# ilyakurdyukov/jpeg-quantsmooth

Measured on AMD Instinct MI355X. Metric: 8x8 blocks/s at q=3 niter=3, higher is better.
Workload: dtype f32

## Files before the change

### include/jpegqs_hip.h

```cpp
#ifndef JPEGQS_HIP_H
#define JPEGQS_HIP_H

#include <stddef.h>
#include <stdint.h>

#ifdef __cplusplus
extern "C" {
#endif

#define QS_HIP_MAXC 4

enum {
	QS_HIP_OK = 0,
	QS_HIP_ENODEV = -1,
	QS_HIP_EINVAL = -2,
	QS_HIP_ENOMEM = -3,
	QS_HIP_ENOTSUP = -4
};


typedef struct {
	int32_t ncomp;
	int32_t colorspace;
	int32_t image_width, image_height;
// ... 120 lines not shown
		int wblk, int hblk, int flags, int luma, int final_clamp, void *stream);
int qs_hip_smooth_plane_next(const void *d_consts, int16_t *d_coef, const uint8_t *d_plane, uint8_t *d_plane_next,
		int wblk, int hblk, int flags, int luma, int final_clamp, int rep_top, int rep_bot, void *stream);
int qs_hip_smooth_rows(const void *d_consts, int16_t *d_coef, const uint8_t *d_plane,
		int wblk, int hblk, int row0, int row1, int flags, int luma, int final_clamp, void *stream);

#define QS_HIP_MAX_PLANES 56
typedef struct {
	const void *d_consts;
	int16_t *d_coef;
	uint8_t *d_plane;
	int32_t *d_status;
	int32_t wblk, hblk, luma;
	int32_t band;
} qs_hip_plane_ref;
int qs_hip_idct_planes(const qs_hip_plane_ref *refs, int n, int first, void *stream);
int qs_hip_smooth_planes(const qs_hip_plane_ref *refs, int n, int flags, int final_clamp, void *stream);
int qs_hip_smooth_planes_next(const qs_hip_plane_ref *refs, uint8_t *const *d_plane_next, int n, int flags,
		int final_clamp, void *stream);

int qs_hip_joint_plane(const void *d_consts, int16_t *d_coef, const uint8_t *d_plane,
		const uint8_t *d_luma_lowres, int wblk, int hblk,
		int rebalance, int final_clamp, void *stream);
int qs_hip_lowq_plane(const void *d_consts, int16_t *d_coef, const uint8_t *d_plane,
		int wblk, int hblk, int rebalance, int final_clamp, void *stream);
int qs_hip_downsample_plane(const uint8_t *d_luma, int ywblk, int yhblk, uint8_t *d_lowres,
		int lwblk, int lhblk, int ws, int hs, void *stream);
size_t qs_hip_upsample_pitch(int image_width, int ws);
size_t qs_hip_upsample_bytes(int image_width, int image_height, int ws, int hs);
int qs_hip_upsample_plane(const uint8_t *d_chroma, const uint8_t *d_luma_lowres, int cwblk,
// ... 15 lines not shown
```

### jpeg-quantsmooth_amd/bands.py

```python
from __future__ import annotations

import os
from dataclasses import dataclass


_LIB = None


def _lib():
    global _LIB
    if _LIB is None:
        try:
            from .hipqs import HipQS
            _LIB = HipQS()
        except (OSError, RuntimeError, ImportError):
            _LIB = False
    return _LIB or None


def _band_rows_py(hblk: int, world: int, rank: int, align: int = 1):
    if hblk < 0 or world < 1 or not 0 <= rank < world or align < 1:
        raise ValueError("band_rows: bad argument")
    units = (hblk + align - 1) // align
    a, b = units * rank // world * align, units * (rank + 1) // world * align
# ... 162 lines not shown
        for w in dist.batch_isend_irecv(ops):
            w.wait()
    for dst_y, buf in recvs:
        view(dst_y).copy_(buf)


def run_bands_batched(engines, topo: BandTopology, niter: int, exchange_many) -> None:
    for it in range(niter):
        for e in engines:
            e.idct(it == 0, topo.rep_top, topo.rep_bot)
        exchange_many()
        for e in engines:
            e.smooth(it == niter - 1)


def run_bands_batched_sets(hip, engines, topo: BandTopology, niter: int, exchange_many, stream=None, mark=None, fused=True) -> None:
    band = (1 if topo.up is not None else 0) | (2 if topo.down is not None else 0)
    flags = engines[0].flags
    s = stream if stream is not None else engines[0]._s()
    if fused:
        for e in engines:
            e.ensure_plane2()
    for it in range(niter):
        if it == 0 or not fused:
            refs = hip.plane_refs([(e.cst.data_ptr(), e.coef.data_ptr(), e.plane.data_ptr(), e.status.data_ptr(),
                                    e.wblk, e.hblk, e.luma, band) for e in engines])
            hip.idct_planes(refs, it == 0, s)
        exchange_many()
        nxt = fused and it < niter - 1
        refs = hip.plane_refs([(e.cst.data_ptr(), e.coef.data_ptr(), e.plane.data_ptr(), e.status.data_ptr(),
                                e.wblk, e.hblk, e.luma, band, e.plane2.data_ptr() if nxt else None) for e in engines])
        if mark:
            mark(0)
        hip.smooth_planes(refs, flags, it == niter - 1, s)
        if mark:
            mark(1)
        if nxt:
            for e in engines:
                e.plane, e.plane2 = e.plane2, e.plane


def run_band_edge_first(hip, e, topo: BandTopology, niter: int, exchange, main, side, torch) -> None:
    if e.hblk < 3:
        return run_bands_batched_sets(hip, [e], topo, niter, exchange, stream=main.cuda_stream)
    e.ensure_plane2()
    band_top = 1 if topo.up is not None else 0
    band_bot = 2 if topo.down is not None else 0
    pitch, wb, hb = e.pitch, e.wblk, e.hblk
    row_bytes = wb * 128

    def views(cur, nxt):
        c0, p0 = e.coef.data_ptr(), cur.data_ptr()
        n0 = nxt.data_ptr() if nxt is not None else None
        at = lambda base, r: base + r * 8 * pitch if base is not None else None
        top = (e.cst.data_ptr(), c0, p0, e.status.data_ptr(), wb, 1, e.luma, band_top | 2, n0)
        bot = (e.cst.data_ptr(), c0 + (hb - 1) * row_bytes, at(p0, hb - 1), e.status.data_ptr(), wb, 1, e.luma, 1 | band_bot, at(n0, hb - 1))
        mid = (e.cst.data_ptr(), c0 + row_bytes, at(p0, 1), e.status.data_ptr(), wb, hb - 2, e.luma, 3, at(n0, 1))
        return hip.plane_refs([top, bot]), hip.plane_refs([mid])
    ev_main, ev_edge = torch.cuda.Event(), torch.cuda.Event()
    whole = hip.plane_refs([(e.cst.data_ptr(), e.coef.data_ptr(), e.plane.data_ptr(), e.status.data_ptr(), wb, hb, e.luma, band_top | band_bot)])
    hip.idct_planes(whole, True, main.cuda_stream)
    ev_main.record(main)
    side.wait_event(ev_main)
    with torch.cuda.stream(side):
        exchange()
    for it in range(niter):
        last = it == niter - 1
        edge, mid = views(e.plane, None if last else e.plane2)
        if it:
            side.wait_event(ev_main)
        hip.smooth_planes(edge, e.flags, last, side.cuda_stream)
        ev_edge_now = torch.cuda.Event(); ev_edge_now.record(side)
        if it:
            main.wait_event(ev_edge)
        hip.smooth_planes(mid, e.flags, last, main.cuda_stream)
        ev_main = torch.cuda.Event(); ev_main.record(main)
        ev_edge = ev_edge_now
        if not last:
            e.plane, e.plane2 = e.plane2, e.plane
            with torch.cuda.stream(side):
                exchange()
    main.wait_event(ev_edge)

# ... 379 lines not shown
```

### jpeg-quantsmooth_amd/csrc/qs_batch.cpp

```cpp
#include <functional>
#include <list>
#include <system_error>

#include "qs_jobint.h"

using namespace qsx;
using namespace qsj;

namespace {

static bool job_couplable(const qs_hip_job* job, int flags, int niter) {
  static const bool off = getenv("QS_HIP_NO_COUPLE") != nullptr;
  if (off || niter < 1 || (flags & QS_LOW_QUALITY) || !job_needs_lowres(job, flags)) return false;
  for (int ci = 0; ci < 3; ++ci) {
    if (!job->has_quant[ci]) return false;
    int acc = 0;
    for (int i = 0; i < 64; ++i) acc |= job->quant[ci][i];
    if (acc <= 1 || acc >= 0x800) return false;
  }
  return true;
}

struct ComputeSlots {
  std::mutex mu;
// ... 91 lines not shown
    for (int g = 0; g < G; ++g)
      for (int ci = 0; ci < 3; ++ci)
        host_pieces(jobs[which[g]], ci, 0, jobs[which[g]]->hblk[ci], cj[g].coef_off[ci], pieces);
    HIP_TRY(upload_pieces(coef.p, pieces, coef_bytes, s, stage));
  }
  HIP_TRY(hipMemsetAsync(status.p, 0, (size_t)G * 3 * sizeof(int32_t), s));
  ComputeSlot slot(current_device());

  auto coef_of = [&](int g, int ci) { return reinterpret_cast<int16_t*>(coef.as<char>() + cj[g].coef_off[ci]); };
  std::vector<unsigned char> cur((size_t)G * 3, 0);
  auto plane_at = [&](int g, int ci, int which_) {
    return px.as<uint8_t>() + cj[g].px_off[ci] + (which_ ? plane_stride(jobs[which[g]]->wblk[ci], jobs[which[g]]->hblk[ci]) : 0);
  };
  auto plane_of = [&](int g, int ci) { return plane_at(g, ci, cur[(size_t)g * 3 + ci]); };
  auto lowres_of = [&](int g) { return cj[g].sub ? px.as<uint8_t>() + cj[g].l_off : plane_of(g, 0); };
  auto make_set = [&](QsPlaneSet& set, int ci0, int ci1, const std::function<bool(int, int)>& next) {
    memset(&set, 0, sizeof set);
    int w = 0, n = 0;
    for (int g = 0; g < G; ++g)
      for (int ci = ci0; ci < ci1; ++ci, ++n) {
        const qs_hip_job* job = jobs[which[g]];
        set.wave0[n] = w;
        w += (job->wblk[ci] * job->hblk[ci] + 63) / 64;
        QsPlaneRef& R = set.ref[n];
        R.cst = cst.as<QsConsts>() + cj[g].cst[ci];
        R.coef = coef_of(g, ci);
        R.plane = plane_of(g, ci);
        R.plane_next = next(g, ci) ? plane_at(g, ci, !cur[(size_t)g * 3 + ci]) : nullptr;
        R.status = status.as<int32_t>() + g * 3 + ci;
        R.wblk = job->wblk[ci]; R.hblk = job->hblk[ci]; R.pitch = qs_plane_pitch(job->wblk[ci]);
        R.mode = QS_PLANE_REP_TOP | QS_PLANE_REP_BOT | (comp_rebalance(job, ci, flags) ? QS_PLANE_REBALANCE : 0);
      }
    set.n = n;
    for (int i = n; i < QS_MAX_PLANES + 2; ++i) set.wave0[i] = w;
  };
  auto flip = [&](int ci0, int ci1, const std::function<bool(int, int)>& next) {
    for (int g = 0; g < G; ++g) for (int ci = ci0; ci < ci1; ++ci) if (next(g, ci)) cur[(size_t)g * 3 + ci] ^= 1;
  };
  const std::function<bool(int, int)> none = [](int, int) { return false; }, all = [](int, int) { return true; };
  QsPlaneSet set;

  make_set(set, 0, 1, none);
  qs_launch_idct_set(set, 1, s);
  for (int it = 0; it < niter; ++it) {
    make_set(set, 0, 1, all);
    qs_launch_smooth_set(set, diag, it == niter - 1, s);
    flip(0, 1, all);
  }
  for (int g = 0; g < G; ++g) {
    const qs_hip_job* job = jobs[which[g]];
    if (cj[g].sub)
      qs_launch_downsample(plane_of(g, 0), job->wblk[0], job->hblk[0], lowres_of(g), job->wblk[1], job->hblk[1],
                           job->hsamp[0], job->vsamp[0], s);
  }

  QsPlaneAux lowres;
  memset(&lowres, 0, sizeof lowres);
  for (int g = 0; g < G; ++g) lowres.p[2 * g] = lowres.p[2 * g + 1] = lowres_of(g);
  bool any_up = false;
  for (int g = 0; g < G; ++g) any_up |= cj[g].upsample;
  const std::function<bool(int, int)> ups = [&](int g, int) { return cj[g].upsample; };
  make_set(set, 1, 3, none);
  qs_launch_idct_set(set, 1, s);
  for (int it = 0; it < niter; ++it) {
    const std::function<bool(int, int)>& next = it < niter - 1 ? all : ups;
    make_set(set, 1, 3, next);
    if (joint)
      qs_launch_joint_set(set, lowres, 0, 0, s);
    qs_launch_smooth_set(set, diag, it == niter - 1, s);
    flip(1, 3, next);
  }
  if (any_up) {
    for (int g = 0; g < G; ++g) {
      if (!cj[g].upsample) continue;
      const qs_hip_job* job = jobs[which[g]];
      const int ws = job->hsamp[0], hs = job->vsamp[0];
      const int w1 = (job->image_width + ws - 1) / ws, h1 = (job->image_height + hs - 1) / hs;
      const size_t pitch = qs_hip_upsample_pitch(job->image_width, ws);
      for (int k = 0; k < 2; ++k) {
        uint8_t* opx = upx.as<uint8_t>() + cj[g].upx_off[k];
        int16_t* oc = reinterpret_cast<int16_t*>(upc.as<char>() + cj[g].upc_off[k]);
// ... 198 lines not shown
```

### jpeg-quantsmooth_amd/csrc/qs_devfn.h

```cpp
#pragma once
#include <hip/hip_runtime.h>
#include <stdint.h>
#include "qs_device.h"

__device__ __forceinline__ int f2i_x86(float v) {
  return (v >= -2147483648.0f && v < 2147483648.0f) ? (int)v : (int)0x80000000;
}

__device__ __forceinline__ float round_half_away(float x) {
  float t = __builtin_truncf(x);
  float fr = __builtin_fabsf(x - t);
  return fr >= 0.5f ? t + __builtin_copysignf(1.0f, x) : t;
}

__device__ __forceinline__ void interval(int c, int div, int x1, int sh, int& orig, int& lo, int& hi) {
  int a = ((x1 * c) >> 16) + c;
  a = (int)(((uint32_t)a << sh) + 0x4000u) >> 15;
  a *= div;
  const int d0 = (div - 1) >> 1, d1 = div >> 1;
  orig = a;
  hi = a + (a < 0 ? d1 : d0);
  lo = a - (a > 0 ? d1 : d0);
}


__device__ __forceinline__ int qs_set_find(const QsPlaneSet& set, int w) {
  int lo = 0, hi = set.n - 1;
  while (lo < hi) {
    const int mid = (lo + hi + 1) >> 1;
    if (set.wave0[mid] <= w) lo = mid; else hi = mid - 1;
  }
  return lo;
}
```

### jpeg-quantsmooth_amd/csrc/qs_device.h

```cpp
#pragma once
#include <stdint.h>

#define QS_APRON_X 16
#define QS_LDS_PITCH 65
#define QS_TAB_MAX 272

enum {
  QS_DIAGONALS = 1, QS_JOINT_YUV = 2, QS_UPSAMPLE_UV = 4, QS_LOW_QUALITY = 8,
  QS_NO_REBALANCE = 16, QS_NO_REBALANCE_UV = 32, QS_TRANSCODE = 64
};

struct QsConsts {
  int32_t nat[64];
  int32_t q[64];
  int32_t qraw[64];
  int32_t x1[64];
  int32_t x2[64];
  float   range[64];
  int32_t qn[64], x1n[64], x2n[64];
  int32_t tab_size;
  int32_t pad[15];
  float   tab[64 * QS_TAB_MAX];
  int32_t rec[64][4];
};
// ... 14 lines not shown
}

#define QS_MAX_PLANES 56
struct QsPlaneRef {
  const QsConsts* cst;
  int16_t* coef;
  uint8_t* plane;
  int32_t* status;
  int32_t wblk, hblk, pitch;
  int32_t mode;
  uint8_t* plane_next;
};
enum {
  QS_PLANE_REBALANCE = 1,
  QS_PLANE_REP_TOP = 2,
  QS_PLANE_REP_BOT = 4
};
struct QsPlaneAux {
  const uint8_t* p[QS_MAX_PLANES];
};
struct QsPlaneSet {
  int32_t n, pad;
  int32_t wave0[QS_MAX_PLANES + 2];
  QsPlaneRef ref[QS_MAX_PLANES];
};
```

### jpeg-quantsmooth_amd/csrc/qs_device_job.cpp

```cpp
#include "qs_common.h"
#include "qs_device_job.h"

#include <algorithm>
#include <new>
#include <vector>

namespace {

size_t align_up(size_t n) { return (n + 255) & ~(size_t)255; }

struct DevComp {
  bool modified = false;
  bool passes = false;
  bool fuse = false;
  bool upsample = false;
  int iters = 0, extra = 0;
  size_t off_cst = 0, off_status = 0, off_plane = 0, off_plane2 = 0, off_snap = 0;
  bool snap = false;
};

struct DevPlan {
  int todo = 0;
  int niter = 0;
  int need_lowres = 0;
// ... 331 lines not shown
  return QS_HIP_OK;
}

int run_sets(qs_hip_job* const* jobs, int njobs, int flags, const BatchPlan& B, char* ws, hipStream_t s) {
  struct Id { int job, ci; };
  std::vector<unsigned char> cur((size_t)njobs * QS_HIP_MAXC, 0);
  auto plane_at = [&](const Id& d, int which) {
    const DevComp& C = B.P[d.job].c[d.ci];
    return reinterpret_cast<uint8_t*>(ws + B.region[d.job] + (which ? C.off_plane2 : C.off_plane));
  };
  auto plane_of = [&](const Id& d) { return plane_at(d, cur[(size_t)d.job * QS_HIP_MAXC + d.ci]); };
  auto lowres_of = [&](int i) {
    return B.P[i].llow_own ? reinterpret_cast<uint8_t*>(ws + B.region[i] + B.P[i].off_llow) : plane_of(Id{i, 0});
  };
  const int diag = (flags & QS_DIAGONALS) != 0;
  auto stage = [&](const std::vector<Id>& ids, bool idct, bool joint, int final_clamp, auto next) {
    for (size_t c0 = 0; c0 < ids.size(); c0 += QS_MAX_PLANES) {
      QsPlaneSet set;
      QsPlaneAux aux;
      memset(&set, 0, sizeof set);
      memset(&aux, 0, sizeof aux);
      const int n = (int)std::min<size_t>(QS_MAX_PLANES, ids.size() - c0);
      int w = 0;
      for (int k = 0; k < n; ++k) {
        const Id& d = ids[c0 + k];
        const qs_hip_job* job = jobs[d.job];
        const DevComp& C = B.P[d.job].c[d.ci];
        set.wave0[k] = w;
        w += (job->wblk[d.ci] * job->hblk[d.ci] + 63) / 64;
        QsPlaneRef& R = set.ref[k];
        R.cst = reinterpret_cast<const QsConsts*>(ws + B.region[d.job] + C.off_cst);
        R.coef = job->coef[d.ci];
        R.plane = plane_of(d);
        R.plane_next = !idct && next(d) ? plane_at(d, !cur[(size_t)d.job * QS_HIP_MAXC + d.ci]) : nullptr;
        R.status = reinterpret_cast<int32_t*>(ws + B.region[d.job] + C.off_status);
        R.wblk = job->wblk[d.ci]; R.hblk = job->hblk[d.ci]; R.pitch = qs_plane_pitch(job->wblk[d.ci]);
        const int rebalance = !(flags & QS_NO_REBALANCE) && (comp_luma(job, d.ci) || !(flags & QS_NO_REBALANCE_UV));
        R.mode = QS_PLANE_REP_TOP | QS_PLANE_REP_BOT | (rebalance ? QS_PLANE_REBALANCE : 0);
        aux.p[k] = lowres_of(d.job);
      }
      set.n = n;
      for (int k = n; k < QS_MAX_PLANES + 2; ++k) set.wave0[k] = w;
      if (idct) {
        qs_launch_idct_set(set, 1, s);
      } else {
        if (joint) qs_launch_joint_set(set, aux, 0, 0, s);
        qs_launch_smooth_set(set, diag, final_clamp, s);
      }
    }
    if (!idct)
      for (const Id& d : ids) if (next(d)) cur[(size_t)d.job * QS_HIP_MAXC + d.ci] ^= 1;
  };

  std::vector<Id> first, chroma;
  for (int i = 0; i < njobs; ++i) {
    if (B.route[i] == ROUTE_SET) for (int ci = 0; ci < jobs[i]->ncomp; ++ci) first.push_back({i, ci});
    if (B.route[i] == ROUTE_COUPLED) { first.push_back({i, 0}); chroma.push_back({i, 1}); chroma.push_back({i, 2}); }
  }
  int niter = 0;
  for (int i = 0; i < njobs; ++i) if (B.route[i] != ROUTE_SEQ) niter = B.P[i].niter;
  const auto none = [](const Id&) { return false; };

  stage(first, true, false, 0, none);
  for (int it = 0; it < niter; ++it) {
    const bool last = it == niter - 1;
    stage(first, false, false, last, [&](const Id& d) { return !last || B.route[d.job] == ROUTE_COUPLED; });
  }
  if (chroma.empty()) return QS_HIP_OK;
  for (int i = 0; i < njobs; ++i) {
    if (B.route[i] != ROUTE_COUPLED || !B.P[i].llow_own) continue;
    const qs_hip_job* job = jobs[i];
    if (int r = qs_hip_downsample_plane(plane_of(Id{i, 0}), job->wblk[0], job->hblk[0], lowres_of(i), job->wblk[1],
                                        job->hblk[1], job->hsamp[0], job->vsamp[0], s)) return r;
  }
  const bool joint = (flags & QS_JOINT_YUV) != 0;
  stage(chroma, true, false, 0, none);
  for (int it = 0; it < niter; ++it) {
    const bool last = it == niter - 1;
    stage(chroma, false, joint, last, [&](const Id& d) { return !last || B.P[d.job].c[d.ci].upsample; });
  }
  for (int i = 0; i < njobs; ++i) {
    if (B.route[i] != ROUTE_COUPLED || !B.P[i].up) continue;
    qs_hip_job* job = jobs[i];
    const int ws0 = job->hsamp[0], hs0 = job->vsamp[0];
    uint8_t* px = reinterpret_cast<uint8_t*>(ws + B.region[i] + B.P[i].off_px);
    for (int ci = 1; ci < 3; ++ci) {
      if (int r = qs_hip_upsample_plane(plane_of(Id{i, ci}), lowres_of(i), job->wblk[ci], plane_of(Id{i, 0}),
                                        job->wblk[0], job->hblk[0], px, job->image_width, job->image_height, ws0, hs0, s))
        return r;
      if (int r = qs_hip_fdct_plane(px, qs_hip_upsample_pitch(job->image_width, ws0), job->coef_up[ci - 1],
                                    job->wblk[0], job->hblk[0], s)) return r;
    }
  }
  return QS_HIP_OK;
// ... 143 lines not shown
```

### jpeg-quantsmooth_amd/csrc/qs_fused.cpp

```cpp
#include <list>

#include "qs_jobint.h"

using namespace qsx;
using namespace qsj;


namespace {
static size_t plane_stride(int wb, int hb) { return (qs_hip_plane_bytes(wb, hb) + 255) & ~(size_t)255; }
struct FPlane { int job, ci, wb, hb, cst; size_t coef_off, px_off, cbytes; int src_row0, keep0, keep1; };
struct FGroup {
  std::vector<FPlane> planes;
  std::vector<int> jobs;
  DevBuf coef, px, cst, status;
  PinnedBuf stage;
  std::vector<QsConsts> hc;
  PinnedBuf hstatus;
  Download down;
  hipStream_t s = nullptr;
  size_t blocks = 0, coef_bytes = 0;
  std::vector<hipEvent_t> it_ev;
  long long units = 0;
  PinnedBuf hstatus0;
  hipEvent_t ev_status0 = nullptr;
// ... 150 lines not shown
    set.n = np;
    int w = 0;
    for (int i = 0; i < np; ++i) {
      const FPlane& P = G.planes[i];
      set.wave0[i] = w;
      w += (P.wb * P.hb + 63) / 64;
      QsPlaneRef& R = set.ref[i];
      R.cst = G.cst.as<QsConsts>() + P.cst;
      R.coef = reinterpret_cast<int16_t*>(G.coef.as<char>() + P.coef_off);
      R.plane = G.px.as<uint8_t>() + P.px_off;
      R.status = G.status.as<int32_t>() + i;
      R.wblk = P.wb; R.hblk = P.hb; R.pitch = qs_plane_pitch(P.wb);
      R.mode = QS_PLANE_REP_TOP | QS_PLANE_REP_BOT | (comp_rebalance(jobs[P.job], P.ci, flags) ? QS_PLANE_REBALANCE : 0);
    }
    for (int i = np; i < QS_MAX_PLANES + 2; ++i) set.wave0[i] = w;
    qs_launch_idct_set(set, 1, G.s);
    if (plan) {
      if (!G.hstatus0.alloc((size_t)np * sizeof(int32_t))) return qs_fail(QS_HIP_ENOMEM, "out of pinned host memory");
      HIP_TRY(hipMemcpyAsync(G.hstatus0.p, G.status.p, (size_t)np * sizeof(int32_t), hipMemcpyDeviceToHost, G.s));
      HIP_TRY(hipEventCreateWithFlags(&G.ev_status0, hipEventDisableTiming));
      HIP_TRY(hipEventRecord(G.ev_status0, G.s));
    }
    for (int it = 0; it < niter; ++it) {
      for (int i = 0; i < np; ++i) {
        uint8_t* a = G.px.as<uint8_t>() + G.planes[i].px_off;
        uint8_t* b = a + plane_stride(G.planes[i].wb, G.planes[i].hb);
        set.ref[i].plane = (it & 1) ? b : a;
        set.ref[i].plane_next = it == niter - 1 ? nullptr : (it & 1) ? a : b;
      }
      qs_launch_smooth_set(set, diag, it == niter - 1, G.s);
      if (plan) {
        hipEvent_t e = nullptr;
        HIP_TRY(hipEventCreateWithFlags(&e, hipEventDisableTiming));
        G.it_ev.push_back(e);
        HIP_TRY(hipEventRecord(e, G.s));
      }
    }
    if (plan) for (const FPlane& P : G.planes) G.units += (long long)(P.keep1 - P.keep0) * jobs[P.job]->vsamp[P.ci];
    HIP_TRY(hipGetLastError());
    if (G.tev[1]) HIP_TRY(hipEventRecord(G.tev[1], G.s));
    if (!G.hstatus.alloc((size_t)np * sizeof(int32_t))) return qs_fail(QS_HIP_ENOMEM, "out of pinned host memory");
    HIP_TRY(hipMemcpyAsync(G.hstatus.p, G.status.p, (size_t)np * sizeof(int32_t), hipMemcpyDeviceToHost, G.s));
    HIP_TRY(G.down.issue(G.coef.p, coef_bytes, G.s, rows_active()));
    if (G.tev[2]) HIP_TRY(hipEventRecord(G.tev[2], G.s));
    if (!G.stage.p) for (int ji : G.jobs) if (split[ji]) defer[ji] = 1;
// ... 114 lines not shown
```

### jpeg-quantsmooth_amd/csrc/qs_kernels.hip

```cpp
#include <hip/hip_runtime.h>
#include <stdint.h>
#include <stdlib.h>
#include "qs_device.h"



__device__ __forceinline__ void wave_lds_sync() {
  __builtin_amdgcn_fence(__ATOMIC_RELEASE, "wavefront");
  __builtin_amdgcn_wave_barrier();
  __builtin_amdgcn_fence(__ATOMIC_ACQUIRE, "wavefront");
}

__device__ __forceinline__ uint32_t mulc(uint32_t a, int c) {
  return (uint32_t)__mul24((int)a, c);
}

__device__ __forceinline__ uint32_t lshl13_add(uint32_t x, uint32_t b) {
  uint32_t r;
  asm("v_lshl_add_u32 %0, %1, 13, %2" : "=v"(r) : "v"(x), "v"(b));
  return r;
}

__device__ __forceinline__ void idct8(uint32_t (&v)[8], uint32_t bias) {
  uint32_t z1, z2, z3, z4, z5, t0, t1, t2, t3, e0, e1, e2, e3;
// ... 85 lines not shown
                 int rep_top, int rep_bot, int blk) {
  const int by = blk / wblk, bx = blk - by * wblk;
  idct_pass1(ws);
  uint8_t* org = plane + (size_t)(by * 8 + 1) * pitch + QS_APRON_X + bx * 8;
#pragma unroll
  for (int y = 0; y < 8; ++y) {
    uint32_t row[8]; int o[8];
#pragma unroll
    for (int j = 0; j < 8; ++j) row[j] = ws[y * 8 + j];
    idct_pass2_row(row, o);
    store_pixel_row(org, pitch, y, o, bx, by, wblk, hblk, rep_top, rep_bot);
  }
}

__device__ __forceinline__ void
idct_block_to_plane(const QsConsts* __restrict__ cst, int16_t* __restrict__ coef,
                    uint8_t* __restrict__ plane, int wblk, int hblk, int pitch,
                    int first, int rep_top, int rep_bot, int* __restrict__ status, int blk) {
  uint4* cp = reinterpret_cast<uint4*>(coef) + (size_t)blk * 8;
  uint32_t ws[64];
#pragma unroll
  for (int j = 0; j < 8; ++j) {
    uint4 v = cp[j];
    uint32_t d[4] = {v.x, v.y, v.z, v.w};
#pragma unroll
    for (int c = 0; c < 4; ++c) {
      ws[j * 8 + c * 2] = (uint32_t)(int32_t)(int16_t)(d[c] & 0xffff);
      ws[j * 8 + c * 2 + 1] = (uint32_t)((int32_t)d[c] >> 16);
    }
  }
  if (first) {
    int bad = 0;
#pragma unroll
    for (int j = 0; j < 8; ++j) {
      uint32_t d[4];
#pragma unroll
      for (int c = 0; c < 4; ++c) {
        int lo = (int32_t)ws[j * 8 + c * 2] * cst->qraw[j * 8 + c * 2];
        int hi = (int32_t)ws[j * 8 + c * 2 + 1] * cst->qraw[j * 8 + c * 2 + 1];
        bad |= ((unsigned)(lo + 0x800) > 0xfffu) | ((unsigned)(hi + 0x800) > 0xfffu);
        lo = (int16_t)lo; hi = (int16_t)hi;
        ws[j * 8 + c * 2] = (uint32_t)lo; ws[j * 8 + c * 2 + 1] = (uint32_t)hi;
        d[c] = ((uint32_t)lo & 0xffffu) | ((uint32_t)hi << 16);
      }
      cp[j] = make_uint4(d[0], d[1], d[2], d[3]);
    }
    if (bad) atomicOr(status, 1);
  }
  idct_ws_to_plane(ws, plane, wblk, hblk, pitch, rep_top, rep_bot, blk);
}

__global__ void __launch_bounds__(256)
qs_idct_plane_kernel(const QsConsts* __restrict__ cst, int16_t* __restrict__ coef,
                     uint8_t* __restrict__ plane, int wblk, int hblk, int pitch,
                     int first, int rep_top, int rep_bot, int* __restrict__ status) {
  const int blk = blockIdx.x * 256 + threadIdx.x;
  if (blk >= wblk * hblk) return;
  idct_block_to_plane(cst, coef, plane, wblk, hblk, pitch, first, rep_top, rep_bot, status, blk);
}

#include "qs_devfn.h"

__global__ void __launch_bounds__(256)
qs_idct_set_kernel(const QsPlaneSet set, int first) {
  const int w = __builtin_amdgcn_readfirstlane((int)(blockIdx.x * 4 + (threadIdx.x >> 6)));
  if (w >= set.wave0[set.n]) return;
  const int i = qs_set_find(set, w);
  const QsPlaneRef& r = set.ref[i];
  const int blk = (w - set.wave0[i]) * 64 + (threadIdx.x & 63);
  if (blk >= r.wblk * r.hblk) return;
  idct_block_to_plane(r.cst, r.coef, r.plane, r.wblk, r.hblk, r.pitch, first,
                      r.mode & QS_PLANE_REP_TOP, r.mode & QS_PLANE_REP_BOT, r.status, blk);
}



typedef int16_t __attribute__((may_alias)) lds_i16;
__device__ __forceinline__ int lds_coef(const uint32_t* col, int i) {
  const lds_i16* p = reinterpret_cast<const lds_i16*>(col + (i >> 1) * QS_LDS_PITCH) + (i & 1);
  return *p;
}
__device__ __forceinline__ void lds_set_coef(uint32_t* col, int i, int v) {
  lds_i16* p = reinterpret_cast<lds_i16*>(col + (i >> 1) * QS_LDS_PITCH) + (i & 1);
  *p = (lds_i16)v;
}

static_assert(QS_LDS_PITCH * 4 == 260, "the literal offsets below assume a 260-byte row pitch");
// ... 143 lines not shown
#pragma unroll
    for (int c = 0; c < 4; ++c) {
      int lo = (int16_t)(d[c] & 0xffff), hi = (int32_t)d[c] >> 16;
      lo *= cst->qraw[j * 8 + c * 2]; hi *= cst->qraw[j * 8 + c * 2 + 1];
      d[c] = ((uint32_t)lo & 0xffffu) | ((uint32_t)hi << 16);
    }
    p[i] = make_uint4(d[0], d[1], d[2], d[3]);
  }
}

#include "qs_launch.h"

void qs_launch_idct_plane(const QsConsts* cst, int16_t* coef, uint8_t* plane, int wblk, int hblk,
                          int first, int rep_top, int rep_bot, int* status, hipStream_t s) {
  const int nblk = wblk * hblk;
  hipLaunchKernelGGL(qs_idct_plane_kernel, dim3((nblk + 255) / 256), dim3(256), 0, s,
                     cst, coef, plane, wblk, hblk, qs_plane_pitch(wblk), first, rep_top, rep_bot, status);
}

#define QS_DP_WAVES 4
static int qs_dp_waves(int groups) {
  static const int on = [] { const char* v = getenv("QS_HIP_DP"); return v ? atoi(v) : 1; }();
  static const int lim = [] { const char* v = getenv("QS_HIP_DP_GROUPS"); return v ? atoi(v) : 768; }();
  static const int lim2 = [] { const char* v = getenv("QS_HIP_DP_GROUPS2"); return v ? atoi(v) : 1536; }();
  if (!on) return 0;
  return groups <= lim ? QS_DP_WAVES : groups <= lim2 ? 2 : 0;
}

void qs_launch_smooth_plane(const QsConsts* cst, int16_t* coef, const uint8_t* plane, uint8_t* plane_next, int rep_top, int rep_bot,
                            int wblk, int hblk, int diag, int rebalance, int final_clamp, int blk_begin, int blk_end, hipStream_t s) {
  const int n = blk_end - blk_begin;
  if (n <= 0) return;
// ... 51 lines not shown
```

### jpeg-quantsmooth_amd/csrc/qs_planes.cpp

```cpp
#include "qs_common.h"


static int check_plane_args(const void* a, const void* b, int wblk, int hblk, const char* who) {
  if (!a || !b) return qs_fail(QS_HIP_EINVAL, "%s: null device pointer", who);
  if (wblk <= 0 || hblk <= 0 || (long long)wblk * hblk > (1ll << 28))
    return qs_fail(QS_HIP_EINVAL, "%s: bad plane size %dx%d blocks", who, wblk, hblk);
  return 0;
}


extern "C" int qs_hip_band_rows(int hblk, int nbands, int band, int align, int* row0, int* row1) {
  if (hblk < 0 || nbands < 1 || band < 0 || band >= nbands || align < 1 || !row0 || !row1)
    return qs_fail(QS_HIP_EINVAL, "qs_hip_band_rows: bad argument");
  const long long units = ((long long)hblk + align - 1) / align;
  const long long a = units * band / nbands * align, b = units * (band + 1) / nbands * align;
  *row0 = (int)(a < hblk ? a : hblk);
  *row1 = (int)(b < hblk ? b : hblk);
  return QS_HIP_OK;
}

extern "C" int qs_hip_colour_band_rows(int hblk_luma, int hblk_chroma, int v_samp, int nbands, int band,
                                       int* y0, int* y1, int* c0, int* c1) {
  if (v_samp < 1 || !y0 || !y1 || !c0 || !c1) return qs_fail(QS_HIP_EINVAL, "qs_hip_colour_band_rows: bad argument");
  if (int r = qs_hip_band_rows(hblk_chroma, nbands, band, 1, c0, c1)) return r;
// ... 69 lines not shown
  int w = 0;
  for (int i = 0; i < n; ++i) {
    const qs_hip_plane_ref& r = refs[i];
    if (int e = check_plane_args(r.d_coef, r.d_plane, r.wblk, r.hblk, who)) return e;
    if (!r.d_consts) return qs_fail(QS_HIP_EINVAL, "%s: null consts", who);
    set.wave0[i] = w;
    w += (r.wblk * r.hblk + 63) / 64;
    QsPlaneRef& R = set.ref[i];
    R.cst = static_cast<const QsConsts*>(r.d_consts);
    R.coef = r.d_coef; R.plane = r.d_plane; R.status = r.d_status;
    R.plane_next = next ? next[i] : nullptr;
    if (R.plane_next && R.plane_next == r.d_plane)
      return qs_fail(QS_HIP_EINVAL, "%s: d_plane_next must be a different buffer (other blocks still read d_plane)", who);
    R.wblk = r.wblk; R.hblk = r.hblk; R.pitch = qs_plane_pitch(r.wblk);
    R.mode = ((!(flags & QS_NO_REBALANCE) && (r.luma || !(flags & QS_NO_REBALANCE_UV))) ? QS_PLANE_REBALANCE : 0) |
             ((r.band & 1) ? 0 : QS_PLANE_REP_TOP) | ((r.band & 2) ? 0 : QS_PLANE_REP_BOT);
  }
  for (int i = n; i < QS_MAX_PLANES + 2; ++i) set.wave0[i] = w;
  return QS_HIP_OK;
}

extern "C" int qs_hip_idct_planes(const qs_hip_plane_ref* refs, int n, int first, void* stream) {
  QsPlaneSet set;
  if (int r = build_plane_set(refs, nullptr, n, 0, set, "qs_hip_idct_planes")) return r;
  if (first)
    for (int i = 0; i < n; ++i)
      if (!refs[i].d_status) return qs_fail(QS_HIP_EINVAL, "qs_hip_idct_planes: first pass needs d_status");
  qs_launch_idct_set(set, first, static_cast<hipStream_t>(stream));
  return launch_status("qs_hip_idct_planes");
}

// ... 97 lines not shown
```

### jpeg-quantsmooth_amd/csrc/qs_smooth_dp_kernel.inc

```
template <bool DIAG, int NW>
__global__ void __launch_bounds__(64 * NW, 3)
#ifdef QS_DP_SET
QS_DP_KERNEL_NAME(const QsPlaneSet set, int final_clamp) {
  const int gw = (int)blockIdx.x;
  if (gw >= set.wave0[set.n]) return;
  const int pi = qs_set_find(set, gw);
  const QsConsts* __restrict__ cst = set.ref[pi].cst;
  int16_t* __restrict__ coef = set.ref[pi].coef;
  const uint8_t* __restrict__ plane = set.ref[pi].plane;
  const int wblk = set.ref[pi].wblk, pitch = set.ref[pi].pitch;
  const int rebalance = set.ref[pi].mode & QS_PLANE_REBALANCE;
  const int nblk = wblk * set.ref[pi].hblk;
  const int base = (gw - set.wave0[pi]) * 64;
#else
QS_DP_KERNEL_NAME(const QsConsts* __restrict__ cst, int16_t* __restrict__ coef,
                  const uint8_t* __restrict__ plane, uint8_t* __restrict__ plane_next, int rep,
                  int wblk, int hblk, int pitch,
                  int rebalance, int final_clamp, int blk_begin, int blk_end) {
  const int nblk = blk_end;
  const int base = blk_begin + (int)blockIdx.x * 64;
#endif
  __shared__ uint32_t lds[32 * QS_LDS_PITCH];
  __shared__ long long reb_part[NW][64][2];
  __shared__ uint32_t chg_sh[3];
  __shared__ uint32_t ws_sh[64 * 64];
  const int lane = threadIdx.x & 63;
  const int wave = __builtin_amdgcn_readfirstlane((int)(threadIdx.x >> 6));
  uint32_t* col = lds + lane;
  if (blockDim.x != 64 * NW) __builtin_trap();
  if (base >= nblk) return;
  const int nvec = min(64, nblk - base) * 8;

  uint4* gsrc = reinterpret_cast<uint4*>(coef) + (size_t)base * 8;
  {
    const int m0 = (lane & 7) * 4;
#pragma unroll
    for (int j = 0; j < 8; ++j) {
      if (j % NW != wave) continue;
      const int idx = j * 64 + lane;
      uint4 v = make_uint4(0, 0, 0, 0);
      if (idx < nvec) v = gsrc[idx];
      uint32_t* dst = lds + m0 * QS_LDS_PITCH + (j * 8 + (lane >> 3));
      dst[0] = v.x; dst[QS_LDS_PITCH] = v.y; dst[2 * QS_LDS_PITCH] = v.z; dst[3 * QS_LDS_PITCH] = v.w;
    }
  }
  const int blk = min(base + lane, nblk - 1);
  const int by = blk / wblk, bx = blk - by * wblk;
  const uint8_t* org = plane + (size_t)(by * 8 + 1) * pitch + QS_APRON_X + bx * 8;
// ... 280 lines not shown
```

### jpeg-quantsmooth_amd/csrc/qs_smooth_kernel.inc

```
template <bool DIAG>
__global__ void __launch_bounds__(64 * QS_WAVES_PER_WG, QS_SMOOTH_MIN_WAVES)
#ifdef QS_SMOOTH_SET
QS_SMOOTH_KERNEL_NAME(const QsPlaneSet set, int final_clamp) {
  __shared__ uint32_t lds_all[QS_WAVES_PER_WG][32 * QS_LDS_PITCH];
#if QS_STASH
  __shared__ uint32_t stash_all[QS_WAVES_PER_WG][2 * 8 * 64];
#endif
  const int lane = threadIdx.x & 63, wave = threadIdx.x >> 6;
  uint32_t* lds = lds_all[wave];
  uint32_t* col = lds + lane;
  const int gw = __builtin_amdgcn_readfirstlane((int)(blockIdx.x * QS_WAVES_PER_WG + wave));
  if (gw >= set.wave0[set.n]) return;
  const int pi = qs_set_find(set, gw);
  const QsConsts* __restrict__ cst = set.ref[pi].cst;
  int16_t* __restrict__ coef = set.ref[pi].coef;
  const uint8_t* __restrict__ plane = set.ref[pi].plane;
  const int wblk = set.ref[pi].wblk, hblk = set.ref[pi].hblk, pitch = set.ref[pi].pitch;
  const int rebalance = set.ref[pi].mode & QS_PLANE_REBALANCE;
  const int nblk = wblk * hblk;
  const int base = (gw - set.wave0[pi]) * 64;
  (void)hblk;
#else
QS_SMOOTH_KERNEL_NAME(const QsConsts* __restrict__ cst, int16_t* __restrict__ coef,
                       const uint8_t* __restrict__ plane, uint8_t* __restrict__ plane_next, int rep,
// ... 6 lines not shown
  const int lane = threadIdx.x & 63, wave = threadIdx.x >> 6;
  uint32_t* lds = lds_all[wave];
  uint32_t* col = lds + lane;
  const int nblk = blk_end;
  const int base = blk_begin + (blockIdx.x * QS_WAVES_PER_WG + wave) * 64;
#endif
  if (base >= nblk) return;
  const int tail_prio = __builtin_amdgcn_readfirstlane(
      (gridDim.x > QS_RESIDENT_WG && blockIdx.x >= (gridDim.x / QS_RESIDENT_WG) * QS_RESIDENT_WG) ? 1 : 0);
  const int nvec = min(64, nblk - base) * 8;
#ifdef QS_STAGGER
  { unsigned hwid; asm volatile("s_getreg_b32 %0, hwreg(HW_REG_HW_ID)" : "=s"(hwid)); if (hwid & 1u) __builtin_amdgcn_s_sleep(QS_STAGGER); }
#endif

  uint4* gsrc = reinterpret_cast<uint4*>(coef) + (size_t)base * 8;
  {
    const int m0 = (lane & 7) * 4;
#pragma unroll
    for (int j = 0; j < 8; ++j) {
      const int idx = j * 64 + lane;
      uint4 v = make_uint4(0, 0, 0, 0);
      if (idx < nvec) v = gsrc[idx];
      uint32_t* dst = lds + m0 * QS_LDS_PITCH + (j * 8 + (lane >> 3));
      dst[0] = v.x; dst[QS_LDS_PITCH] = v.y; dst[2 * QS_LDS_PITCH] = v.z; dst[3 * QS_LDS_PITCH] = v.w;
    }
  }

  const int blk = min(base + lane, nblk - 1);
  const int by = blk / wblk, bx = blk - by * wblk;
  const uint8_t* org = plane + (size_t)(by * 8 + 1) * pitch + QS_APRON_X + bx * 8;
// ... 312 lines not shown
```

Baseline: 273.9 million.

## Defer first-pass dequantized coefficient writeback into first smooth pass; coalesce IDCT loads

The first IDCT pass no longer writes dequantized coefficients back to global memory when a smoothing pass follows. Instead, the first smooth kernel re-dequantizes the raw coefficients on load using a per-plane QS_PLANE_QUANT mode bit. The IDCT kernel is also restructured to load each wave's 64 blocks coalesced and transpose them through LDS, rather than having each thread read its own block. This removes one full coefficient write pass and improves load coalescing, at the cost of extra mode plumbing through every host path and a small dequant multiply in the first smooth pass.

```diff
diff --git a/include/jpegqs_hip.h b/include/jpegqs_hip.h
--- a/include/jpegqs_hip.h
+++ b/include/jpegqs_hip.h
@@ -158,6 +158,8 @@
 	int32_t wblk, hblk, luma;
 	int32_t band;
 } qs_hip_plane_ref;
+#define QS_HIP_PLANE_DEFER 4
+#define QS_HIP_FIRST_DEFER 2
 int qs_hip_idct_planes(const qs_hip_plane_ref *refs, int n, int first, void *stream);
 int qs_hip_smooth_planes(const qs_hip_plane_ref *refs, int n, int flags, int final_clamp, void *stream);
 int qs_hip_smooth_planes_next(const qs_hip_plane_ref *refs, uint8_t *const *d_plane_next, int n, int flags,
diff --git a/jpeg-quantsmooth_amd/bands.py b/jpeg-quantsmooth_amd/bands.py
--- a/jpeg-quantsmooth_amd/bands.py
+++ b/jpeg-quantsmooth_amd/bands.py
@@ -200,6 +200,10 @@
             e.smooth(it == niter - 1)
 
 
+def defer_bit() -> int:
+    return 0 if os.environ.get("QS_BANDS_DEFER", "1") == "0" else 4
+
+
 def run_bands_batched_sets(hip, engines, topo: BandTopology, niter: int, exchange_many, stream=None, mark=None, fused=True) -> None:
     band = (1 if topo.up is not None else 0) | (2 if topo.down is not None else 0)
     flags = engines[0].flags
@@ -208,14 +212,15 @@
         for e in engines:
             e.ensure_plane2()
     for it in range(niter):
+        q = defer_bit() if it == 0 else 0
         if it == 0 or not fused:
             refs = hip.plane_refs([(e.cst.data_ptr(), e.coef.data_ptr(), e.plane.data_ptr(), e.status.data_ptr(),
-                                    e.wblk, e.hblk, e.luma, band) for e in engines])
+                                    e.wblk, e.hblk, e.luma, band | q) for e in engines])
             hip.idct_planes(refs, it == 0, s)
         exchange_many()
         nxt = fused and it < niter - 1
         refs = hip.plane_refs([(e.cst.data_ptr(), e.coef.data_ptr(), e.plane.data_ptr(), e.status.data_ptr(),
-                                e.wblk, e.hblk, e.luma, band, e.plane2.data_ptr() if nxt else None) for e in engines])
+                                e.wblk, e.hblk, e.luma, band | q, e.plane2.data_ptr() if nxt else None) for e in engines])
         if mark:
             mark(0)
         hip.smooth_planes(refs, flags, it == niter - 1, s)
@@ -235,16 +240,17 @@
     pitch, wb, hb = e.pitch, e.wblk, e.hblk
     row_bytes = wb * 128
 
-    def views(cur, nxt):
+    def views(cur, nxt, q):
         c0, p0 = e.coef.data_ptr(), cur.data_ptr()
         n0 = nxt.data_ptr() if nxt is not None else None
         at = lambda base, r: base + r * 8 * pitch if base is not None else None
-        top = (e.cst.data_ptr(), c0, p0, e.status.data_ptr(), wb, 1, e.luma, band_top | 2, n0)
-        bot = (e.cst.data_ptr(), c0 + (hb - 1) * row_bytes, at(p0, hb - 1), e.status.data_ptr(), wb, 1, e.luma, 1 | band_bot, at(n0, hb - 1))
-        mid = (e.cst.data_ptr(), c0 + row_bytes, at(p0, 1), e.status.data_ptr(), wb, hb - 2, e.luma, 3, at(n0, 1))
+        top = (e.cst.data_ptr(), c0, p0, e.status.data_ptr(), wb, 1, e.luma, band_top | 2 | q, n0)
+        bot = (e.cst.data_ptr(), c0 + (hb - 1) * row_bytes, at(p0, hb - 1), e.status.data_ptr(), wb, 1, e.luma, 1 | band_bot | q, at(n0, hb - 1))
+        mid = (e.cst.data_ptr(), c0 + row_bytes, at(p0, 1), e.status.data_ptr(), wb, hb - 2, e.luma, 3 | q, at(n0, 1))
         return hip.plane_refs([top, bot]), hip.plane_refs([mid])
     ev_main, ev_edge = torch.cuda.Event(), torch.cuda.Event()
-    whole = hip.plane_refs([(e.cst.data_ptr(), e.coef.data_ptr(), e.plane.data_ptr(), e.status.data_ptr(), wb, hb, e.luma, band_top | band_bot)])
+    whole = hip.plane_refs([(e.cst.data_ptr(), e.coef.data_ptr(), e.plane.data_ptr(), e.status.data_ptr(), wb, hb, e.luma,
+                             band_top | band_bot | (defer_bit() if niter > 0 else 0))])
     hip.idct_planes(whole, True, main.cuda_stream)
     ev_main.record(main)
     side.wait_event(ev_main)
@@ -252,7 +258,7 @@
         exchange()
     for it in range(niter):
         last = it == niter - 1
-        edge, mid = views(e.plane, None if last else e.plane2)
+        edge, mid = views(e.plane, None if last else e.plane2, defer_bit() if it == 0 else 0)
         if it:
             side.wait_event(ev_main)
         hip.smooth_planes(edge, e.flags, last, side.cuda_stream)
diff --git a/jpeg-quantsmooth_amd/csrc/qs_batch.cpp b/jpeg-quantsmooth_amd/csrc/qs_batch.cpp
--- a/jpeg-quantsmooth_amd/csrc/qs_batch.cpp
+++ b/jpeg-quantsmooth_amd/csrc/qs_batch.cpp
@@ -129,7 +129,7 @@
   };
   auto plane_of = [&](int g, int ci) { return plane_at(g, ci, cur[(size_t)g * 3 + ci]); };
   auto lowres_of = [&](int g) { return cj[g].sub ? px.as<uint8_t>() + cj[g].l_off : plane_of(g, 0); };
-  auto make_set = [&](QsPlaneSet& set, int ci0, int ci1, const std::function<bool(int, int)>& next) {
+  auto make_set = [&](QsPlaneSet& set, int ci0, int ci1, const std::function<bool(int, int)>& next, bool quant = false) {
     memset(&set, 0, sizeof set);
     int w = 0, n = 0;
     for (int g = 0; g < G; ++g)
@@ -144,7 +144,8 @@
         R.plane_next = next(g, ci) ? plane_at(g, ci, !cur[(size_t)g * 3 + ci]) : nullptr;
         R.status = status.as<int32_t>() + g * 3 + ci;
         R.wblk = job->wblk[ci]; R.hblk = job->hblk[ci]; R.pitch = qs_plane_pitch(job->wblk[ci]);
-        R.mode = QS_PLANE_REP_TOP | QS_PLANE_REP_BOT | (comp_rebalance(job, ci, flags) ? QS_PLANE_REBALANCE : 0);
+        R.mode = QS_PLANE_REP_TOP | QS_PLANE_REP_BOT | (comp_rebalance(job, ci, flags) ? QS_PLANE_REBALANCE : 0) |
+                 (quant ? QS_PLANE_QUANT : 0);
       }
     set.n = n;
     for (int i = n; i < QS_MAX_PLANES + 2; ++i) set.wave0[i] = w;
@@ -155,10 +156,11 @@
   const std::function<bool(int, int)> none = [](int, int) { return false; }, all = [](int, int) { return true; };
   QsPlaneSet set;
 
-  make_set(set, 0, 1, none);
+  const bool defer_y = niter > 0;
+  make_set(set, 0, 1, none, defer_y);
   qs_launch_idct_set(set, 1, s);
   for (int it = 0; it < niter; ++it) {
-    make_set(set, 0, 1, all);
+    make_set(set, 0, 1, all, defer_y && it == 0);
     qs_launch_smooth_set(set, diag, it == niter - 1, s);
     flip(0, 1, all);
   }
@@ -175,11 +177,12 @@
   bool any_up = false;
   for (int g = 0; g < G; ++g) any_up |= cj[g].upsample;
   const std::function<bool(int, int)> ups = [&](int g, int) { return cj[g].upsample; };
-  make_set(set, 1, 3, none);
+  const bool defer_c = niter > 0 && !joint;
+  make_set(set, 1, 3, none, defer_c);
   qs_launch_idct_set(set, 1, s);
   for (int it = 0; it < niter; ++it) {
     const std::function<bool(int, int)>& next = it < niter - 1 ? all : ups;
-    make_set(set, 1, 3, next);
+    make_set(set, 1, 3, next, defer_c && it == 0);
     if (joint)
       qs_launch_joint_set(set, lowres, 0, 0, s);
     qs_launch_smooth_set(set, diag, it == niter - 1, s);
diff --git a/jpeg-quantsmooth_amd/csrc/qs_devfn.h b/jpeg-quantsmooth_amd/csrc/qs_devfn.h
--- a/jpeg-quantsmooth_amd/csrc/qs_devfn.h
+++ b/jpeg-quantsmooth_amd/csrc/qs_devfn.h
@@ -24,6 +24,24 @@
 }
 
 
+__device__ __forceinline__ void qs_load_qraw8(const QsConsts* __restrict__ cst, int e, int (&q)[8]) {
+  const int4* qp = reinterpret_cast<const int4*>(cst->qraw) + e * 2;
+  const int4 a = qp[0], b = qp[1];
+  q[0] = a.x; q[1] = a.y; q[2] = a.z; q[3] = a.w; q[4] = b.x; q[5] = b.y; q[6] = b.z; q[7] = b.w;
+}
+template <bool CHECK>
+__device__ __forceinline__ uint4 qs_dequant8(uint4 v, const int (&q)[8], int& bad) {
+  uint32_t d[4] = {v.x, v.y, v.z, v.w};
+#pragma unroll
+  for (int c = 0; c < 4; ++c) {
+    const int lo = (int32_t)(int16_t)(d[c] & 0xffff) * q[c * 2];
+    const int hi = ((int32_t)d[c] >> 16) * q[c * 2 + 1];
+    if (CHECK) bad |= ((unsigned)(lo + 0x800) > 0xfffu) | ((unsigned)(hi + 0x800) > 0xfffu);
+    d[c] = ((uint32_t)lo & 0xffffu) | ((uint32_t)hi << 16);
+  }
+  return make_uint4(d[0], d[1], d[2], d[3]);
+}
+
 __device__ __forceinline__ int qs_set_find(const QsPlaneSet& set, int w) {
   int lo = 0, hi = set.n - 1;
   while (lo < hi) {
diff --git a/jpeg-quantsmooth_amd/csrc/qs_device.h b/jpeg-quantsmooth_amd/csrc/qs_device.h
--- a/jpeg-quantsmooth_amd/csrc/qs_device.h
+++ b/jpeg-quantsmooth_amd/csrc/qs_device.h
@@ -52,7 +52,8 @@
 enum {
   QS_PLANE_REBALANCE = 1,
   QS_PLANE_REP_TOP = 2,
-  QS_PLANE_REP_BOT = 4
+  QS_PLANE_REP_BOT = 4,
+  QS_PLANE_QUANT = 8
 };
 struct QsPlaneAux {
   const uint8_t* p[QS_MAX_PLANES];
diff --git a/jpeg-quantsmooth_amd/csrc/qs_device_job.cpp b/jpeg-quantsmooth_amd/csrc/qs_device_job.cpp
--- a/jpeg-quantsmooth_amd/csrc/qs_device_job.cpp
+++ b/jpeg-quantsmooth_amd/csrc/qs_device_job.cpp
@@ -369,7 +369,7 @@
     return B.P[i].llow_own ? reinterpret_cast<uint8_t*>(ws + B.region[i] + B.P[i].off_llow) : plane_of(Id{i, 0});
   };
   const int diag = (flags & QS_DIAGONALS) != 0;
-  auto stage = [&](const std::vector<Id>& ids, bool idct, bool joint, int final_clamp, auto next) {
+  auto stage = [&](const std::vector<Id>& ids, bool idct, bool joint, int final_clamp, auto next, bool quant = false) {
     for (size_t c0 = 0; c0 < ids.size(); c0 += QS_MAX_PLANES) {
       QsPlaneSet set;
       QsPlaneAux aux;
@@ -391,7 +391,7 @@
         R.status = reinterpret_cast<int32_t*>(ws + B.region[d.job] + C.off_status);
         R.wblk = job->wblk[d.ci]; R.hblk = job->hblk[d.ci]; R.pitch = qs_plane_pitch(job->wblk[d.ci]);
         const int rebalance = !(flags & QS_NO_REBALANCE) && (comp_luma(job, d.ci) || !(flags & QS_NO_REBALANCE_UV));
-        R.mode = QS_PLANE_REP_TOP | QS_PLANE_REP_BOT | (rebalance ? QS_PLANE_REBALANCE : 0);
+        R.mode = QS_PLANE_REP_TOP | QS_PLANE_REP_BOT | (rebalance ? QS_PLANE_REBALANCE : 0) | (quant ? QS_PLANE_QUANT : 0);
         aux.p[k] = lowres_of(d.job);
       }
       set.n = n;
@@ -416,10 +416,11 @@
   for (int i = 0; i < njobs; ++i) if (B.route[i] != ROUTE_SEQ) niter = B.P[i].niter;
   const auto none = [](const Id&) { return false; };
 
-  stage(first, true, false, 0, none);
+  const bool defer = niter > 0;
+  stage(first, true, false, 0, none, defer);
   for (int it = 0; it < niter; ++it) {
     const bool last = it == niter - 1;
-    stage(first, false, false, last, [&](const Id& d) { return !last || B.route[d.job] == ROUTE_COUPLED; });
+    stage(first, false, false, last, [&](const Id& d) { return !last || B.route[d.job] == ROUTE_COUPLED; }, defer && it == 0);
   }
   if (chroma.empty()) return QS_HIP_OK;
   for (int i = 0; i < njobs; ++i) {
@@ -429,10 +430,11 @@
                                         job->hblk[1], job->hsamp[0], job->vsamp[0], s)) return r;
   }
   const bool joint = (flags & QS_JOINT_YUV) != 0;
-  stage(chroma, true, false, 0, none);
+  const bool defer_c = defer && !joint;
+  stage(chroma, true, false, 0, none, defer_c);
   for (int it = 0; it < niter; ++it) {
     const bool last = it == niter - 1;
-    stage(chroma, false, joint, last, [&](const Id& d) { return !last || B.P[d.job].c[d.ci].upsample; });
+    stage(chroma, false, joint, last, [&](const Id& d) { return !last || B.P[d.job].c[d.ci].upsample; }, defer_c && it == 0);
   }
   for (int i = 0; i < njobs; ++i) {
     if (B.route[i] != ROUTE_COUPLED || !B.P[i].up) continue;
diff --git a/jpeg-quantsmooth_amd/csrc/qs_fused.cpp b/jpeg-quantsmooth_amd/csrc/qs_fused.cpp
--- a/jpeg-quantsmooth_amd/csrc/qs_fused.cpp
+++ b/jpeg-quantsmooth_amd/csrc/qs_fused.cpp
@@ -188,6 +188,8 @@
       R.mode = QS_PLANE_REP_TOP | QS_PLANE_REP_BOT | (comp_rebalance(jobs[P.job], P.ci, flags) ? QS_PLANE_REBALANCE : 0);
     }
     for (int i = np; i < QS_MAX_PLANES + 2; ++i) set.wave0[i] = w;
+    const bool quant = niter > 0;
+    if (quant) for (int i = 0; i < np; ++i) set.ref[i].mode |= QS_PLANE_QUANT;
     qs_launch_idct_set(set, 1, G.s);
     if (plan) {
       if (!G.hstatus0.alloc((size_t)np * sizeof(int32_t))) return qs_fail(QS_HIP_ENOMEM, "out of pinned host memory");
@@ -203,6 +205,7 @@
         set.ref[i].plane_next = it == niter - 1 ? nullptr : (it & 1) ? a : b;
       }
       qs_launch_smooth_set(set, diag, it == niter - 1, G.s);
+      if (it == 0) for (int i = 0; i < np; ++i) set.ref[i].mode &= ~QS_PLANE_QUANT;
       if (plan) {
         hipEvent_t e = nullptr;
         HIP_TRY(hipEventCreateWithFlags(&e, hipEventDisableTiming));
diff --git a/jpeg-quantsmooth_amd/csrc/qs_kernels.hip b/jpeg-quantsmooth_amd/csrc/qs_kernels.hip
--- a/jpeg-quantsmooth_amd/csrc/qs_kernels.hip
+++ b/jpeg-quantsmooth_amd/csrc/qs_kernels.hip
@@ -2,6 +2,7 @@
 #include <stdint.h>
 #include <stdlib.h>
 #include "qs_device.h"
+#include "qs_devfn.h"
 
 
 
@@ -123,63 +124,77 @@
 }
 
 __device__ __forceinline__ void
-idct_block_to_plane(const QsConsts* __restrict__ cst, int16_t* __restrict__ coef,
-                    uint8_t* __restrict__ plane, int wblk, int hblk, int pitch,
-                    int first, int rep_top, int rep_bot, int* __restrict__ status, int blk) {
-  uint4* cp = reinterpret_cast<uint4*>(coef) + (size_t)blk * 8;
-  uint32_t ws[64];
+idct_wave_to_plane(const QsConsts* __restrict__ cst, int16_t* __restrict__ coef,
+                   uint8_t* __restrict__ plane, int wblk, int hblk, int pitch,
+                   int first, int defer, int rep_top, int rep_bot, int* __restrict__ status, int base, uint32_t* lds) {
+  const int lane = threadIdx.x & 63;
+  const int nblk = wblk * hblk;
+  const int nvec = min(64, nblk - base) * 8;
+  uint4* gsrc = reinterpret_cast<uint4*>(coef) + (size_t)base * 8;
+  uint4 v[8];
 #pragma unroll
   for (int j = 0; j < 8; ++j) {
-    uint4 v = cp[j];
-    uint32_t d[4] = {v.x, v.y, v.z, v.w};
-#pragma unroll
-    for (int c = 0; c < 4; ++c) {
-      ws[j * 8 + c * 2] = (uint32_t)(int32_t)(int16_t)(d[c] & 0xffff);
-      ws[j * 8 + c * 2 + 1] = (uint32_t)((int32_t)d[c] >> 16);
-    }
+    const int idx = j * 64 + lane;
+    v[j] = make_uint4(0, 0, 0, 0);
+    if (idx < nvec) v[j] = gsrc[idx];
   }
   if (first) {
-    int bad = 0;
-#pragma unroll
-    for (int j = 0; j < 8; ++j) {
-      uint32_t d[4];
-#pragma unroll
-      for (int c = 0; c < 4; ++c) {
-        int lo = (int32_t)ws[j * 8 + c * 2] * cst->qraw[j * 8 + c * 2];
-        int hi = (int32_t)ws[j * 8 + c * 2 + 1] * cst->qraw[j * 8 + c * 2 + 1];
-        bad |= ((unsigned)(lo + 0x800) > 0xfffu) | ((unsigned)(hi + 0x800) > 0xfffu);
-        lo = (int16_t)lo; hi = (int16_t)hi;
-        ws[j * 8 + c * 2] = (uint32_t)lo; ws[j * 8 + c * 2 + 1] = (uint32_t)hi;
-        d[c] = ((uint32_t)lo & 0xffffu) | ((uint32_t)hi << 16);
+    int q[8], bad = 0;
+    qs_load_qraw8(cst, lane & 7, q);
+#pragma unroll
+    for (int j = 0; j < 8; ++j) v[j] = qs_dequant8<true>(v[j], q, bad);
+    if (!defer) {
+#pragma unroll
+      for (int j = 0; j < 8; ++j) {
+        const int idx = j * 64 + lane;
+        if (idx < nvec) gsrc[idx] = v[j];
       }
-      cp[j] = make_uint4(d[0], d[1], d[2], d[3]);
     }
     if (bad) atomicOr(status, 1);
   }
-  idct_ws_to_plane(ws, plane, wblk, hblk, pitch, rep_top, rep_bot, blk);
+  {
+    const int m0 = (lane & 7) * 4;
+#pragma unroll
+    for (int j = 0; j < 8; ++j) {
+      uint32_t* dst = lds + m0 * QS_LDS_PITCH + (j * 8 + (lane >> 3));
+      dst[0] = v[j].x; dst[QS_LDS_PITCH] = v[j].y; dst[2 * QS_LDS_PITCH] = v[j].z; dst[3 * QS_LDS_PITCH] = v[j].w;
+    }
+  }
+  wave_lds_sync();
+  const uint32_t* col = lds + lane;
+  uint32_t ws[64];
+#pragma unroll
+  for (int r = 0; r < 32; ++r) {
+    const uint32_t d = col[r * QS_LDS_PITCH];
+    ws[r * 2] = (uint32_t)(int32_t)(int16_t)(d & 0xffff);
+    ws[r * 2 + 1] = (uint32_t)((int32_t)d >> 16);
+  }
+  if (base + lane < nblk) idct_ws_to_plane(ws, plane, wblk, hblk, pitch, rep_top, rep_bot, base + lane);
 }
 
 __global__ void __launch_bounds__(256)
 qs_idct_plane_kernel(const QsConsts* __restrict__ cst, int16_t* __restrict__ coef,
                      uint8_t* __restrict__ plane, int wblk, int hblk, int pitch,
                      int first, int rep_top, int rep_bot, int* __restrict__ status) {
-  const int blk = blockIdx.x * 256 + threadIdx.x;
-  if (blk >= wblk * hblk) return;
-  idct_block_to_plane(cst, coef, plane, wblk, hblk, pitch, first, rep_top, rep_bot, status, blk);
-}
-
-#include "qs_devfn.h"
+  __shared__ uint32_t lds_all[4][32 * QS_LDS_PITCH];
+  const int wave = threadIdx.x >> 6;
+  const int base = __builtin_amdgcn_readfirstlane((int)(blockIdx.x * 256 + wave * 64));
+  if (base >= wblk * hblk) return;
+  idct_wave_to_plane(cst, coef, plane, wblk, hblk, pitch, first & 1, first & 2, rep_top, rep_bot, status, base, lds_all[wave]);
+}
 
 __global__ void __launch_bounds__(256)
 qs_idct_set_kernel(const QsPlaneSet set, int first) {
-  const int w = __builtin_amdgcn_readfirstlane((int)(blockIdx.x * 4 + (threadIdx.x >> 6)));
+  __shared__ uint32_t lds_all[4][32 * QS_LDS_PITCH];
+  const int wave = threadIdx.x >> 6;
+  const int w = __builtin_amdgcn_readfirstlane((int)(blockIdx.x * 4 + wave));
   if (w >= set.wave0[set.n]) return;
   const int i = qs_set_find(set, w);
   const QsPlaneRef& r = set.ref[i];
-  const int blk = (w - set.wave0[i]) * 64 + (threadIdx.x & 63);
-  if (blk >= r.wblk * r.hblk) return;
-  idct_block_to_plane(r.cst, r.coef, r.plane, r.wblk, r.hblk, r.pitch, first,
-                      r.mode & QS_PLANE_REP_TOP, r.mode & QS_PLANE_REP_BOT, r.status, blk);
+  const int base = (w - set.wave0[i]) * 64;
+  if (base >= r.wblk * r.hblk) return;
+  idct_wave_to_plane(r.cst, r.coef, r.plane, r.wblk, r.hblk, r.pitch, first, r.mode & QS_PLANE_QUANT,
+                     r.mode & QS_PLANE_REP_TOP, r.mode & QS_PLANE_REP_BOT, r.status, base, lds_all[wave]);
 }
 
 
@@ -353,8 +368,9 @@
 void qs_launch_idct_plane(const QsConsts* cst, int16_t* coef, uint8_t* plane, int wblk, int hblk,
                           int first, int rep_top, int rep_bot, int* status, hipStream_t s) {
   const int nblk = wblk * hblk;
+  const int f = first == 3 ? 3 : first ? 1 : 0;
   hipLaunchKernelGGL(qs_idct_plane_kernel, dim3((nblk + 255) / 256), dim3(256), 0, s,
-                     cst, coef, plane, wblk, hblk, qs_plane_pitch(wblk), first, rep_top, rep_bot, status);
+                     cst, coef, plane, wblk, hblk, qs_plane_pitch(wblk), f, rep_top, rep_bot, status);
 }
 
 #define QS_DP_WAVES 4
diff --git a/jpeg-quantsmooth_amd/csrc/qs_planes.cpp b/jpeg-quantsmooth_amd/csrc/qs_planes.cpp
--- a/jpeg-quantsmooth_amd/csrc/qs_planes.cpp
+++ b/jpeg-quantsmooth_amd/csrc/qs_planes.cpp
@@ -107,7 +107,8 @@
       return qs_fail(QS_HIP_EINVAL, "%s: d_plane_next must be a different buffer (other blocks still read d_plane)", who);
     R.wblk = r.wblk; R.hblk = r.hblk; R.pitch = qs_plane_pitch(r.wblk);
     R.mode = ((!(flags & QS_NO_REBALANCE) && (r.luma || !(flags & QS_NO_REBALANCE_UV))) ? QS_PLANE_REBALANCE : 0) |
-             ((r.band & 1) ? 0 : QS_PLANE_REP_TOP) | ((r.band & 2) ? 0 : QS_PLANE_REP_BOT);
+             ((r.band & 1) ? 0 : QS_PLANE_REP_TOP) | ((r.band & 2) ? 0 : QS_PLANE_REP_BOT) |
+             ((r.band & QS_HIP_PLANE_DEFER) ? QS_PLANE_QUANT : 0);
   }
   for (int i = n; i < QS_MAX_PLANES + 2; ++i) set.wave0[i] = w;
   return QS_HIP_OK;
diff --git a/jpeg-quantsmooth_amd/csrc/qs_smooth_dp_kernel.inc b/jpeg-quantsmooth_amd/csrc/qs_smooth_dp_kernel.inc
--- a/jpeg-quantsmooth_amd/csrc/qs_smooth_dp_kernel.inc
+++ b/jpeg-quantsmooth_amd/csrc/qs_smooth_dp_kernel.inc
@@ -32,6 +32,23 @@
   const int nvec = min(64, nblk - base) * 8;
 
   uint4* gsrc = reinterpret_cast<uint4*>(coef) + (size_t)base * 8;
+#ifdef QS_DP_SET
+  if (set.ref[pi].mode & QS_PLANE_QUANT) {
+    const int m0 = (lane & 7) * 4;
+    int q[8], unused = 0;
+    qs_load_qraw8(cst, lane & 7, q);
+#pragma unroll
+    for (int j = 0; j < 8; ++j) {
+      if (j % NW != wave) continue;
+      const int idx = j * 64 + lane;
+      uint4 v = make_uint4(0, 0, 0, 0);
+      if (idx < nvec) v = gsrc[idx];
+      v = qs_dequant8<false>(v, q, unused);
+      uint32_t* dst = lds + m0 * QS_LDS_PITCH + (j * 8 + (lane >> 3));
+      dst[0] = v.x; dst[QS_LDS_PITCH] = v.y; dst[2 * QS_LDS_PITCH] = v.z; dst[3 * QS_LDS_PITCH] = v.w;
+    }
+  } else
+#endif
   {
     const int m0 = (lane & 7) * 4;
 #pragma unroll
diff --git a/jpeg-quantsmooth_amd/csrc/qs_smooth_kernel.inc b/jpeg-quantsmooth_amd/csrc/qs_smooth_kernel.inc
--- a/jpeg-quantsmooth_amd/csrc/qs_smooth_kernel.inc
+++ b/jpeg-quantsmooth_amd/csrc/qs_smooth_kernel.inc
@@ -44,6 +44,22 @@
 #endif
 
   uint4* gsrc = reinterpret_cast<uint4*>(coef) + (size_t)base * 8;
+#ifdef QS_SMOOTH_SET
+  if (set.ref[pi].mode & QS_PLANE_QUANT) {
+    const int m0 = (lane & 7) * 4;
+    int q[8], unused = 0;
+    qs_load_qraw8(cst, lane & 7, q);
+#pragma unroll
+    for (int j = 0; j < 8; ++j) {
+      const int idx = j * 64 + lane;
+      uint4 v = make_uint4(0, 0, 0, 0);
+      if (idx < nvec) v = gsrc[idx];
+      v = qs_dequant8<false>(v, q, unused);
+      uint32_t* dst = lds + m0 * QS_LDS_PITCH + (j * 8 + (lane >> 3));
+      dst[0] = v.x; dst[QS_LDS_PITCH] = v.y; dst[2 * QS_LDS_PITCH] = v.z; dst[3 * QS_LDS_PITCH] = v.w;
+    }
+  } else
+#endif
   {
     const int m0 = (lane & 7) * 4;
 #pragma unroll
```

After: 277.1 million, median of 6. 1.01x the previous value.
